# sunkafei/coffeedb

Hardware: AMD Instinct MI355X
Metric: sa_build_GiB_per_s (higher is better)
Workload: dtype u64

## Files before the change

### coffeedb_amd/csrc/debug_segsort.hip

```cpp
#include <cstdio>
#include <cstring>
#include <mutex>
#include <string>
#include <vector>

#include "../../include/coffeedb_gpu.h"
#include "index_impl.h"
#include "radix_sort.h"

using namespace cdb;

namespace {

std::mutex g_err_mu;
std::string g_err;

template <typename F>
int guarded_hook(const char* who, F&& f) {
    const int rc = guarded_call(g_err_mu, g_err, std::forward<F>(f));
    if (rc != CDB_OK) {
        std::lock_guard<std::mutex> g(g_err_mu);
        std::fprintf(stderr, "%s: %s\n", who, g_err.c_str());
    }
    return rc;
// ... 73 lines not shown
        CallStream cs(device);
        hipStream_t s = cs.s;
        StreamScope sscope(s);
        if (!rs_atomic_rank_ok(s)) throw InternalError("cdb_debug_segsort: needs the one-atomic ranking (internal)");
        const uint32_t cell_tiles_max = tiles + (form == CDB_DEBUG_SEGSORT_TOP_FIRST ? nb * 256u : 0u);
        Guarded k[2], v[2], w[2], eout, ehi, flags;
        for (int q = 0; q < 2; ++q) {
            k[q].alloc(n, 4, s);
            v[q].alloc(n, 4, s);
            w[q].alloc(n, 2, s);
        }
        eout.alloc(n, packed ? 4 : 8, s);
        ehi.alloc(n, 1, s);
        flags.alloc(n, 1, s);
        CDB_HIP(hipMemcpyAsync(k[0].ptr<uint32_t>(), k32, n * 4, hipMemcpyHostToDevice, s));
        CDB_HIP(hipMemcpyAsync(v[0].ptr<uint32_t>(), v32, n * 4, hipMemcpyHostToDevice, s));
        CDB_HIP(hipMemcpyAsync(w[0].ptr<uint16_t>(), w16, n * 2, hipMemcpyHostToDevice, s));
        DevBuf d_segs, d_tile_seg, d_hist, d_starts, edges;
        d_segs.alloc((size_t)nb * sizeof(SegInfo));
        CDB_HIP(hipMemcpyAsync(d_segs.p, segs.data(), (size_t)nb * sizeof(SegInfo), hipMemcpyHostToDevice, s));
        d_tile_seg.alloc((size_t)tiles * sizeof(uint32_t));
        d_hist.alloc((size_t)nb * 8 * 256 * sizeof(uint64_t));
        d_starts.alloc((size_t)nb * 8 * 256 * sizeof(uint64_t));
        edges.alloc((size_t)cell_tiles_max * 256 * sizeof(SegEdge));
        hipLaunchKernelGGL(rs_seg_tilemap_kernel, dim3((unsigned)ceil_div(tiles, 256u)), dim3(256), 0, s, (const SegInfo*)d_segs.as<SegInfo>(), nb, tiles,
                           d_tile_seg.as<uint32_t>());
        SegFinalArgs fin;
        if (packed) {
            fin.elo = eout.ptr<uint32_t>();
            fin.ehi = ehi.ptr<uint8_t>();
        } else {
            fin.eout = eout.ptr<uint64_t>();
        }
        fin.flags = flags.ptr<uint8_t>();
        fin.edges = edges.as<SegEdge>();
        fin.hi_shift = 8;
        fin.low_bits = 8;
        fin.kbase = 2;
        fin.kmagic = 0;
        if (carry) {
            fin.hi_mask = (1u << ehb) - 1u;
            fin.carry_mask = (1u << carry) - 1u;
            fin.carry_shift = 8 + ehb;
        }
        RadixWorkspace ws;
        ws.allow_group = true;
        Profiler prof;
        TopFirstWork tfw;
        uint32_t ncell = 0;
        if (form == CDB_DEBUG_SEGSORT_TOP_FIRST) {
            tfw.alloc(nb * 256u, cell_tiles_max);
            rs_top_first_fin(fin, ehb);
            ncell = radix_sort_top_first<uint16_t>(s, ws, prof, k[0].ptr<uint32_t>(), k[1].ptr<uint32_t>(), v[0].ptr<uint32_t>(), v[1].ptr<uint32_t>(),
                                                   w[0].ptr<uint16_t>(), w[1].ptr<uint16_t>(), n, (const SegInfo*)d_segs.as<SegInfo>(), segs.data(),
                                                   (const uint32_t*)d_tile_seg.as<uint32_t>(), nb, tiles, d_hist.as<unsigned long long>(),
                                                   d_starts.as<unsigned long long>(), tfw, fin, nullptr);
        } else {
            CDB_HIP(hipMemsetAsync(d_hist.p, 0, (size_t)nb * 8 * 256 * sizeof(uint64_t), s));
            hipLaunchKernelGGL((rs_seg_hist_kernel<uint16_t>), dim3((unsigned)ceil_div(tiles, (uint32_t)RS_MSD_HIST_TILES)), dim3(1024), 0, s,
                               (const uint32_t*)k[0].ptr<uint32_t>(), (const uint16_t*)w[0].ptr<uint16_t>(), 1, 5, (const uint32_t*)d_tile_seg.as<uint32_t>(),
                               (const SegInfo*)d_segs.as<SegInfo>(), tiles, d_hist.as<unsigned long long>());
            radix_sort_segmented<uint16_t>(s, ws, prof, k[0].ptr<uint32_t>(), k[1].ptr<uint32_t>(), v[0].ptr<uint32_t>(), v[1].ptr<uint32_t>(),
                                           w[0].ptr<uint16_t>(), w[1].ptr<uint16_t>(), n, (const SegInfo*)d_segs.as<SegInfo>(),
                                           (const uint32_t*)d_tile_seg.as<uint32_t>(), nb, tiles, (const unsigned long long*)d_hist.as<unsigned long long>(),
                                           d_starts.as<unsigned long long>(), 32, 1, fin, nullptr);
        }
        CDB_HIP(hipStreamSynchronize(s));
        radix_check_error(s, ws);
        if (packed) {
            std::vector<uint32_t> lo(n);
            std::vector<uint8_t> hi(n);
            CDB_HIP(hipMemcpyAsync(lo.data(), eout.ptr<uint32_t>(), n * 4, hipMemcpyDeviceToHost, s));
            CDB_HIP(hipMemcpyAsync(hi.data(), ehi.ptr<uint8_t>(), n, hipMemcpyDeviceToHost, s));
            CDB_HIP(hipStreamSynchronize(s));
            for (uint64_t i = 0; i < n; ++i) out_entries[i] = ((uint64_t)hi[i] << 32) | lo[i];
        } else {
            CDB_HIP(hipMemcpyAsync(out_entries, eout.ptr<uint64_t>(), n * 8, hipMemcpyDeviceToHost, s));
        }
        CDB_HIP(hipMemcpyAsync(out_flags, flags.ptr<uint8_t>(), n, hipMemcpyDeviceToHost, s));
// ... 17 lines not shown
```

### coffeedb_amd/csrc/radix_pass.h

```cpp
#pragma once
#include <cstdlib>

#include "common.h"

namespace cdb {

constexpr uint64_t RS_VAL_MASK = (1ull << 54) - 1;
constexpr uint32_t RS_SPIN_LIMIT_GROUPED = 1u << 18;
constexpr uint32_t RS_SPIN_LIMIT_PLAIN = 1u << 22;
constexpr int RS_GROUP = 8;

struct NoVal {};

__device__ __forceinline__ uint64_t rs_ld_status(const uint64_t* p) {
    return __hip_atomic_load(p, __ATOMIC_RELAXED, __HIP_MEMORY_SCOPE_AGENT);
}
__device__ __forceinline__ void rs_st_status(uint64_t* p, uint64_t v) {
    __hip_atomic_store(p, v, __ATOMIC_RELAXED, __HIP_MEMORY_SCOPE_AGENT);
}

template <int IPT_, bool REUSE_, bool EARLYV_, int NT_ = 256, bool NONTEMP_ = false, int MINW_ = 1, int ABL_ = 0,
          int LB_ = 1, bool DMA_ = false, bool ATOMRANK_ = false, bool TICKET_ = true, int LOAD_ = 0, int GROUP_ = 0>
struct RsCfg {
    static constexpr int GROUP = GROUP_;
    static constexpr int LOAD = LOAD_;
    static constexpr bool TICKET = TICKET_;
// ... 93 lines not shown
struct SegShrinkArgs : SegArgs {
    uint8_t* wout8 = nullptr;
};
struct SegEdge {
    unsigned long long first, last;
    unsigned long long pos;
    uint32_t cnt, pad;
};
struct SegFinalArgs : SegArgs {
    uint64_t* eout = nullptr;
    uint32_t* elo = nullptr;
    uint8_t* ehi = nullptr;
    uint8_t* flags = nullptr;
    SegEdge* edges = nullptr;
    int hi_shift = 0;
    int low_bits = 0;
    uint32_t kbase = 2;
    unsigned long long kmagic = 0;
    uint32_t hi_mask = 0xFFFFFFFFu;
    uint32_t carry_mask = 0;
    int carry_shift = 0;
};

struct SegFinalKeepArgs : SegArgs {
    uint8_t* flags = nullptr;
    SegEdge* edges = nullptr;
    int low_bits = 0;
    uint32_t kbase = 2;
    unsigned long long kmagic = 0;
    unsigned long long* tile_sums = nullptr;
    uint32_t sums_tile = 1;
    unsigned long long msd_m = 0;
};

struct SegFinalKeepMsdArgs : SegFinalKeepArgs {};

__device__ __forceinline__ uint64_t rs_pack_key(const uint32_t* __restrict__ s_words, uint32_t li, int nsym, uint32_t base,
                                                uint32_t rem) {
    const uint32_t wi = li >> 2, sel = li & 3u;
    const uint32_t b2 = base * base, b3 = b2 * base;
    const uint32_t pw[5] = {1u, base, b2, b3, b3 * base};
    uint64_t kk = 0;
    uint32_t lo = s_words[wi];
#pragma unroll
    for (int w = 0; w < 4; ++w) {
        const int q = 4 * w;
// ... 14 lines not shown

__device__ __forceinline__ uint64_t rs_doc_upper(const uint64_t* __restrict__ doc_start, uint64_t lo, uint64_t hi,
                                                 uint64_t p) {
    while (lo < hi) {
        const uint64_t mid = lo + (hi - lo + 1) / 2;
        if (doc_start[mid] <= p) lo = mid; else hi = mid - 1;
    }
    return lo;
}

template <typename K_, typename V_, typename Cfg_, typename Gen_, typename W_, typename Seg_>
struct RsTraits {
    using K = K_;
    using V = V_;
    using Cfg = Cfg_;
    using Gen = Gen_;
    using W = W_;
    using Seg = Seg_;
    static constexpr bool GEN = !std::is_same<Gen, NoGen>::value;
    static constexpr bool SEG = !std::is_same<Seg, NoSeg>::value;
    static constexpr bool FINAL = std::is_same<Seg, SegFinalArgs>::value;
    static constexpr bool KEEPM = std::is_same<Seg, SegFinalKeepMsdArgs>::value;
    static constexpr bool KEEP = std::is_same<Seg, SegFinalKeepArgs>::value || KEEPM;
    static constexpr bool FLAGS = FINAL || KEEP;
    static constexpr bool SHRINK = std::is_same<Seg, SegShrinkArgs>::value;
    static constexpr bool HAS_V = !std::is_same<V, NoVal>::value;
    static constexpr bool HAS_W = !std::is_same<W, NoVal>::value;
    using WS = typename std::conditional<HAS_W, W, uint8_t>::type;
    using VS = typename std::conditional<HAS_V, V, uint32_t>::type;
    static constexpr int IPT = Cfg::IPT;
    static constexpr bool REUSE = Cfg::REUSE && HAS_V;
    static constexpr bool EARLYV = (Cfg::EARLYV || REUSE) && HAS_V;
    static constexpr int NT = Cfg::NT;
    static constexpr int NW = NT / 64;
    static constexpr bool NTM = Cfg::NONTEMP;
    static constexpr int TILE = NT * IPT;
    static constexpr int WCHUNK = 64 * IPT;
    static constexpr size_t STAGE_K = sizeof(K) * TILE;
    static constexpr size_t STAGE_V = HAS_V ? sizeof(VS) * TILE : 0;
    static constexpr size_t STAGE_BYTES = REUSE ? (STAGE_K > STAGE_V ? STAGE_K : STAGE_V) : STAGE_K + STAGE_V;
    static constexpr bool GM_PAIR = std::is_same<Gen, TextGenPair>::value;
    static constexpr bool GM_REC = std::is_same<Gen, TextGenRec>::value;
    static constexpr bool BLK = GEN && sizeof(K) == 4 && sizeof(VS) == 4 && IPT == 16 && (NT == 1024 || NT == 512);
    static constexpr uint32_t GEN_TEXTB = ((TILE + RS_GEN_LOOK + 15) / 16) * 16;
    static constexpr uint32_t GEN_DOCS = 1024;
    static constexpr uint32_t GEN_SLOTS = 320;
    static constexpr size_t GEN_BYTES = BLK ? GEN_TEXTB + 512 + GEN_DOCS * 8 + GEN_SLOTS : 16;
    static constexpr uint32_t MAP_OFF = GEN_TEXTB;
    static constexpr uint32_t DOC_OFF = GEN_TEXTB + 512;
    static constexpr uint32_t DOC_CAP = BLK ? GEN_DOCS : (uint32_t)((STAGE_BYTES - DOC_OFF) / 8);
    static constexpr uint32_t SLOT_OFF = GEN_TEXTB + 512 + GEN_DOCS * 8;
    static constexpr bool W32G = GEN && HAS_W && sizeof(WS) == 4;
    static constexpr bool AUX_LDS = HAS_W && !W32G && !KEEPM;
    static constexpr size_t AUX_ELEMS = AUX_LDS ? TILE : 1;
    static constexpr bool LOAD_W = HAS_W && !KEEPM;
    static constexpr bool DMA_PATH = !GEN && Cfg::DMA && HAS_V && EARLYV && sizeof(K) == 8 && (IPT % 4) == 0;

    static_assert(!SHRINK || (std::is_same<W, uint16_t>::value && Cfg::REUSE && !std::is_same<V, NoVal>::value), "shrinking pass: u16 aux words, shared staging");
    static_assert(!SEG || (!GEN && !Cfg::DMA), "segmented passes: materialised records");
    static_assert(!FLAGS || Cfg::REUSE || KEEPM, "flag-writing passes: shared staging (the MSD-first last pass also runs with keys and values staged at once)");
    static_assert(!HAS_W || KEEPM || (Cfg::REUSE && HAS_V && !Cfg::DMA), "the auxiliary byte needs the shared-staging configuration");
    static_assert(!(GM_PAIR || GM_REC) || (BLK && HAS_W), "pair / records generators: 16 Ki tiles with an auxiliary word");
    static_assert(!GEN || EARLYV, "generator pass needs early values");
    static_assert(!GEN || STAGE_BYTES >= (size_t)TILE + RS_GEN_LOOK + 2048, "staging buffer too small for the text tile");
};
template <typename T>
__device__ __forceinline__ uint32_t rs_group_flag(const typename T::Seg& seg, bool head, bool tail, uint64_t kc, uint64_t slot,
                                                  uint32_t carry) {
    uint32_t f = head ? 1u : 0u;
    if (!(head && tail)) {
        const bool exhausted = seg.kmagic ? (kc - __umul64hi(kc, seg.kmagic) * seg.kbase) == 0
                                          : (kc & (uint64_t)(seg.kbase - 1u)) == 0;
        if (!exhausted) f |= 2u;
    }
    f |= carry;
    if (!(T::FINAL && (RS_SEG_ABL & 1))) seg.flags[slot] = (uint8_t)f;
    if constexpr (T::KEEP) {
        if ((f & 2u) && seg.tile_sums) {
            atomicAdd(seg.tile_sums + 2 * (slot / seg.sums_tile), 1ull);
            if (f & 1u) atomicAdd(seg.tile_sums + 2 * (slot / seg.sums_tile) + 1, 1ull);
        }
    }
// ... 63 lines not shown
        sg = seg.tile_seg ? seg.tile_seg[tile] : 0u;
        si = seg.segs[sg];
        tile0 = si.tile_begin;
        base = si.begin + (tile - tile0) * T::TILE;
        seg_n = si.end;
        if constexpr (T::KEEPM) ktop = (uint64_t)si.top * seg.msd_m;
    } else if constexpr (Cfg::GROUP > 0) {
        if (base >= n) return;
    }
    const uint32_t valid = (uint32_t)((seg_n - base) < (uint64_t)T::TILE ? (seg_n - base) : (uint64_t)T::TILE);
    if (s_bad) {
        if constexpr (T::GEN) {
            if (gen.tile_base) return;
        }
        if (tid < 256) rs_st_status(status + tile * 256 + tid, ((uint64_t)epoch << 56) | (2ull << 54));
        return;
    }

    K key[T::IPT];
    VS val[T::EARLYV ? T::IPT : 1];
    WS aux[T::HAS_W ? T::IPT : 1] = {};
    uint32_t gdig[T::GM_REC ? T::IPT / 4 : 1] = {};
    auto digit_of = [&](K k, WS a) -> uint32_t {
        if constexpr (T::HAS_W) {
            if (aux_shift >= 0) return ((uint32_t)a >> aux_shift) & dmask;
        }
        return (uint32_t)(k >> shift) & dmask;
    };
    const uint32_t wbase = wave * T::WCHUNK + lane;
    if constexpr (T::GEN) {
        unsigned char* const gbuf = T::BLK ? s_gen : s_stage;
        uint8_t* s_text = gbuf;
        uint16_t* s_map = reinterpret_cast<uint16_t*>(gbuf + T::MAP_OFF);
        uint64_t* s_docs = reinterpret_cast<uint64_t*>(gbuf + T::DOC_OFF);
        constexpr bool PRELOAD = T::BLK;
        uint4 tw0 = make_uint4(0, 0, 0, 0), tw1 = make_uint4(0, 0, 0, 0);
        bool tw0_ok = false, tw1_ok = false;
        if constexpr (PRELOAD) {
            const uint64_t g0 = base + (uint64_t)tid * 16, g1 = base + (uint64_t)T::TILE + (uint64_t)tid * 16;
            tw0_ok = gen.padded ? (g0 < n + RS_GEN_LOOK) : (g0 + 16 <= n);
            tw1_ok = (uint32_t)tid * 16 < (uint32_t)RS_GEN_LOOK && (gen.padded ? (g1 < n + RS_GEN_LOOK) : (g1 + 16 <= n));
            if (tw0_ok) tw0 = *reinterpret_cast<const uint4*>(gen.text + g0);
            if (tw1_ok) tw1 = *reinterpret_cast<const uint4*>(gen.text + g1);
        }
        const uint64_t dlo = gen.tile_doc[tile], dhi = gen.tile_doc[tile + 1];
        for (int i = tid; i < 256; i += T::NT) s_map[i] = gen.symmap[i];
        if constexpr (T::GM_REC) {
// ... 398 lines not shown
                atomicAdd(err + 1, (uint32_t)used);
                atomicAdd(err + 2, 1u);
            }
            p -= used;
            if (used == 0) {
                __builtin_amdgcn_s_sleep(1);
                if (++spins > (Cfg::GROUP > 0 ? RS_SPIN_LIMIT_GROUPED : RS_SPIN_LIMIT_PLAIN)) {
                    atomicExch(err, 1u);
                    break;
                }
            } else {
                spins = 0;
            }
        }
        rs_st_status(my, tag | (2ull << 54) | (excl + real));
    }
    uint64_t dstart = 0;
    if (tid < 256) {
        if constexpr (T::SEG) dstart = (uint64_t)digit_start[(size_t)sg * seg.start_stride + d];
        else dstart = (uint64_t)digit_start[d];
        s_gbase[d] = (Cfg::ABL & 2) ? base : (prebased ? pre : dstart + excl) - (uint64_t)tstart;
    }
    __syncthreads();
    if constexpr (T::FLAGS) {
        if (tid < 256) {
            SegEdge e;
            e.first = e.last = 0;
            e.pos = dstart + excl;
            e.cnt = (uint32_t)real;
            e.pad = 0;
            if (real) {
                const uint64_t lmask = (1ull << seg.low_bits) - 1ull;
                const uint32_t a = tstart, b = tstart + (uint32_t)real - 1u;
                if constexpr (T::KEEPM) {
                    e.first = ktop + (uint64_t)s_keys[a];
                    e.last = ktop + (uint64_t)s_keys[b];
                } else {
                    e.first = ((uint64_t)s_keys[a] << seg.low_bits) | ((uint64_t)s_aux[T::HAS_W ? a : 0] & lmask);
                    e.last = ((uint64_t)s_keys[b] << seg.low_bits) | ((uint64_t)s_aux[T::HAS_W ? b : 0] & lmask);
                }
            }
            seg.edges[tile * 256 + d] = e;
        }
    }

    if constexpr (!T::REUSE) {
#pragma unroll
        for (int j = 0; j < T::IPT; ++j) {
            const uint32_t i = j * T::NT + tid;
            if (i < valid) {
                const K k = s_keys[i];
                const uint32_t dd = (uint32_t)(k >> shift) & dmask;
                const uint64_t dst = s_gbase[dd] + i;
                if constexpr (T::KEEPM) {
                    bool head = true, tail = true;
                    if (i > 0) head = s_keys[i - 1] != k;
                    if (i + 1 < valid) tail = s_keys[i + 1] != k;
                    const uint64_t kf = ktop + (uint64_t)k;
                    rs_group_flag<T>(seg, head, tail, kf, dst, 0u);
                    rs_store<T::NTM>(kout + dst, (K)(kf >> 8));
                    if constexpr (T::HAS_W) rs_store<T::NTM>(wout + dst, (W)(kf & 0xFFu));
                    rs_store<T::NTM>(vout + dst, (V)s_vals[i]);
                    continue;
                }
                if (!T::GEN || kout) rs_store<T::NTM>(kout + dst, k);
                if constexpr (T::HAS_V) rs_store<T::NTM>(vout + dst, (V)s_vals[i]);
            }
        }
    } else {
        uint8_t dig[T::IPT];
#pragma unroll
        for (int j = 0; j < T::IPT; ++j) {
            const uint32_t i = j * T::NT + tid;
            dig[j] = 0;
            if (i < valid) {
                const K k = s_keys[i];
                uint32_t dd;
                if constexpr (T::KEEPM) dd = (uint32_t)(k >> shift) & dmask;
                else dd = digit_of(k, s_aux[T::HAS_W ? i : 0]);
                if constexpr (T::GM_REC) dd = (uint32_t)s_gen[i];
                dig[j] = (uint8_t)dd;
                if constexpr (T::FLAGS) {
                    const uint32_t lmask = seg.low_bits >= 32 ? 0xFFFFFFFFu : (1u << seg.low_bits) - 1u;
                    uint32_t ac = 0;
                    if constexpr (!T::KEEPM) ac = (uint32_t)s_aux[T::HAS_W ? i : 0] & lmask;
                    bool head = true, tail = true;
                    bool cmp = true;
                    if constexpr (T::FINAL) cmp = !(RS_SEG_ABL & 4);
                    if constexpr (T::KEEPM) {
// ... 78 lines not shown
```

### coffeedb_amd/csrc/radix_sort.h

```cpp
#pragma once
#include <cstdlib>

#include "common.h"
#include "radix_pass.h"

namespace cdb {

constexpr int RS_MAX_PASSES = 16;

template <typename K>
__global__ __launch_bounds__(256) void rs_hist_kernel(const K* __restrict__ keys, uint64_t n, int begin_bit,
                                                      int npass, int dbits, uint32_t last_mask,
                                                      unsigned long long* __restrict__ ghist) {
    __shared__ uint32_t sh[RS_MAX_PASSES * 256];
    for (int i = threadIdx.x; i < npass * 256; i += 256) sh[i] = 0;
    __syncthreads();
    const uint64_t stride = (uint64_t)gridDim.x * 256;
    for (uint64_t i = (uint64_t)blockIdx.x * 256 + threadIdx.x; i < n; i += stride) {
        const K k = keys[i];
#pragma unroll
        for (int p = 0; p < RS_MAX_PASSES; ++p) {
            if (p < npass) {
                uint32_t d = (uint32_t)(k >> (begin_bit + dbits * p)) & ((1u << dbits) - 1u);
                if (p == npass - 1) d &= last_mask;
// ... 51 lines not shown
        if (r >= (1u << 24) || (b2 - 1) * r >= (1ull << 32)) break;
        bool ok = true;
        for (uint64_t a = 0; a < b2 && ok; ++a) ok = ((a * r) >> sh) == a / span;
        if (ok) {
            gen.pair_span = span;
            gen.pair_r = (uint32_t)r;
            gen.pair_s = sh;
            return true;
        }
    }
    return false;
}

static __global__ __launch_bounds__(256) void rs_tiledoc_kernel(const uint64_t* __restrict__ doc_start, uint64_t ndocs,
                                                                uint64_t n, uint64_t tile_elems, uint64_t tiles,
                                                                uint64_t* __restrict__ tile_doc) {
    const uint64_t t = (uint64_t)blockIdx.x * 256 + threadIdx.x;
    if (t > tiles) return;
    const uint64_t p = t * tile_elems < n ? t * tile_elems : n - 1;
    tile_doc[t] = rs_doc_upper(doc_start, 0, ndocs - 1, p);
}


static __global__ __launch_bounds__(256) void rs_seg_edge_fix_kernel(const SegEdge* __restrict__ edges, const uint32_t* __restrict__ tile_seg,
                                                                     const SegInfo* __restrict__ segs, uint32_t tiles,
                                                                     uint8_t* __restrict__ flags, uint32_t kbase, unsigned long long kmagic,
                                                                     unsigned long long* __restrict__ tile_sums = nullptr,
                                                                     uint32_t sums_tile = 1, const uint32_t* __restrict__ err = nullptr) {
    const uint32_t t = blockIdx.x, d = threadIdx.x;
    if (t >= tiles) return;
    if (err && *err) return;
    const SegEdge e = edges[(size_t)t * 256 + d];
    if (!e.cnt) return;
    const SegInfo si = segs[tile_seg ? tile_seg[t] : 0u];
    const uint32_t t0 = si.tile_begin;
    if (t == t0) return;
    uint32_t lo = t0, hi = t;
    if (edges[(size_t)(t - 1) * 256 + d].pos < e.pos) {
        lo = t - 1;
    } else {
        if (edges[(size_t)t0 * 256 + d].pos >= e.pos) return;
        hi = t - 1;
        while (hi - lo > 1) {
            const uint32_t mid = lo + (hi - lo) / 2;
            if (edges[(size_t)mid * 256 + d].pos < e.pos) lo = mid; else hi = mid;
        }
    }
    const SegEdge pe = edges[(size_t)lo * 256 + d];
    if (pe.last != e.first) return;
    const bool exhausted = kmagic ? (e.first - __umul64hi(e.first, kmagic) * kbase) == 0 : (e.first & (uint64_t)(kbase - 1u)) == 0;
    auto change = [&](unsigned long long slot, uint32_t clear, uint32_t set) {
        const uintptr_t a = reinterpret_cast<uintptr_t>(flags + slot);
        unsigned int* w = reinterpret_cast<unsigned int*>(a & ~(uintptr_t)3);
        const uint32_t sh = 8u * (uint32_t)(a & 3u);
        uint32_t before, after;
        if (clear) {
            before = (atomicAnd(w, ~(clear << sh)) >> sh) & 0xFFu;
            after = before & ~clear;
        } else {
            before = (atomicOr(w, set << sh) >> sh) & 0xFFu;
            after = before | set;
        }
        if (tile_sums && before != after) {
            const long long da = (long long)((after >> 1) & 1u) - (long long)((before >> 1) & 1u);
            const long long db = (long long)((after >> 1) & after & 1u) - (long long)((before >> 1) & before & 1u);
            unsigned long long* ts = tile_sums + 2 * (slot / sums_tile);
            if (da) atomicAdd(ts, (unsigned long long)da);
            if (db) atomicAdd(ts + 1, (unsigned long long)db);
        }
    };
    const unsigned long long sb = rs_seg_rotated(si, e.pos), sa_ = rs_seg_rotated(si, e.pos - 1);
    change(sb, 1u, 0u);
    if (!exhausted) {
        change(sb, 0u, 2u);
        change(sa_, 0u, 2u);
    }
}

static __global__ __launch_bounds__(256) void rs_lane_order_probe_kernel(uint32_t* __restrict__ bad) {
    __shared__ uint32_t cnt[4][256];
    __shared__ uint32_t ref[4][256];
    const int tid = threadIdx.x, lane = tid & 63, wave = tid >> 6;
    for (int i = tid; i < 4 * 256; i += 256) {
        (&cnt[0][0])[i] = 0;
        (&ref[0][0])[i] = 0;
    }
    __syncthreads();
    const uint64_t lt_mask = (1ull << lane) - 1ull;
    uint32_t wrong = 0;
    for (uint32_t r = 0; r < 64; ++r) {
        uint32_t h = (blockIdx.x * 64u + r) * 256u + (uint32_t)tid;
        h ^= h >> 16; h *= 0x7feb352du; h ^= h >> 15; h *= 0x846ca68bu; h ^= h >> 16;
        const uint32_t mode = blockIdx.x & 3u;
        const uint32_t d = mode == 0 ? 7u : mode == 1 ? (h & 1u) * 64u : mode == 2 ? (h & 15u) * 4u : (h & 255u);
        const uint32_t got = atomicAdd(&cnt[wave][d], 1u);
        uint64_t m = ~0ull;
#pragma unroll
        for (int b = 0; b < 8; ++b) {
            const bool bit = (d >> b) & 1u;
// ... 409 lines not shown

static __global__ __launch_bounds__(256) void rs_seg_digit_start_kernel(const unsigned long long* __restrict__ hist,
                                                                        const SegInfo* __restrict__ segs, int npass,
                                                                        unsigned long long* __restrict__ starts) {
    __shared__ unsigned long long s[256];
    const uint32_t g = blockIdx.x;
    const int t = threadIdx.x;
    const unsigned long long b0 = segs[g].begin;
    for (int p = 0; p < npass; ++p) {
        const unsigned long long c = hist[((size_t)g * 8 + p) * 256 + t];
        s[t] = c;
        __syncthreads();
        for (int off = 1; off < 256; off <<= 1) {
            const unsigned long long v = t >= off ? s[t - off] : 0;
            __syncthreads();
            s[t] += v;
            __syncthreads();
        }
        starts[((size_t)g * 8 + p) * 256 + t] = b0 + s[t] - c;
        __syncthreads();
    }
}

template <typename W>
void radix_sort_segmented(hipStream_t s, RadixWorkspace& ws, Profiler& prof, uint32_t* k0, uint32_t* k1, uint32_t* v0, uint32_t* v1,
                          W* w0, W* w1, uint64_t m, const SegInfo* d_segs, const uint32_t* d_tile_seg, uint32_t nseg, uint32_t tiles,
                          const unsigned long long* d_hist, unsigned long long* d_starts, int key_bits, int lead, SegFinalArgs fin,
                          SortStats* stats) {
    if (!rs_atomic_rank_ok(s)) throw InternalError("radix_sort_segmented: needs the one-atomic ranking (internal)");
    const int kpass = (int)ceil_div((uint64_t)key_bits, 8);
    const int npass = kpass + lead;
    if (npass < 1 || npass > 8 || kpass < 1) throw InternalError("radix_sort_segmented: unsupported pass count (internal)");
    const int last_bits = key_bits - 8 * (kpass - 1);
    const uint32_t last_mask = (1u << last_bits) - 1u;
    ws.prepare((uint64_t)tiles * RS_SEG_TILE, RS_SEG_TILE, s);
    hipLaunchKernelGGL(rs_seg_digit_start_kernel, dim3(nseg), dim3(256), 0, s, d_hist, d_segs, npass, d_starts);
    SegArgs sa;
    sa.tile_seg = d_tile_seg;
    sa.segs = d_segs;
    sa.tiles = tiles;
    sa.start_stride = 8 * 256;
    static_cast<SegArgs&>(fin) = sa;
    uint32_t* kb[2] = {k0, k1};
    uint32_t* vb[2] = {v0, v1};
    W* wb[2] = {w0, w1};
    int cur = 0;
    const char* wn = sizeof(W) == 1 ? "_w8" : (sizeof(W) == 2 ? "_w16" : "_w32");
    const size_t rec = 8 + sizeof(W);
    for (int p = 0; p < npass; ++p) {
        const uint32_t dmask = p == npass - 1 ? last_mask : 0xFFu;
        const int shift = 8 * (p - lead);
        const int aux_shift = p < lead ? 8 * p : -1;
        const unsigned long long* dstart = d_starts + (size_t)p * 256;
        int t = prof.begin(s);
        if (p == npass - 1) {
            rs_launch_pass_ordered<RsBig<>, W>(s, ws, tiles, kb[cur], kb[cur ^ 1], vb[cur], vb[cur ^ 1], m, shift, dmask, dstart, NoGen(), wb[cur],
                                               wb[cur ^ 1], aux_shift, fin);
            prof.end(t, (std::string("rs_seg_final") + wn + "_t16384").c_str(), m * (rec + (fin.elo ? 6 : 9)), s);
        } else {
            rs_launch_pass_ordered<RsBig<>, W>(s, ws, tiles, kb[cur], kb[cur ^ 1], vb[cur], vb[cur ^ 1], m, shift, dmask, dstart, NoGen(), wb[cur],
                                               wb[cur ^ 1], aux_shift, sa);
            prof.end(t, (std::string("rs_seg_k32_v32") + wn + "_t16384").c_str(), 2 * m * rec, s);
        }
        cur ^= 1;
        if (stats) stats->passes_run++;
    }
    int t = prof.begin(s);
    hipLaunchKernelGGL(rs_seg_edge_fix_kernel, dim3(tiles), dim3(256), 0, s, (const SegEdge*)fin.edges, d_tile_seg, d_segs, tiles,
                       fin.flags, fin.kbase, fin.kmagic, (unsigned long long*)nullptr, 1u, (const uint32_t*)ws.err_ptr());
    prof.end(t, "rs_seg_edge_fix", (uint64_t)tiles * 256 * sizeof(SegEdge), s);
    CDB_HIP(hipGetLastError());
}

constexpr int RS_MSD_HIST_TILES = 32;

template <typename W, bool KEYS = true>
__global__ __launch_bounds__(1024) void rs_seg_hist_kernel(const uint32_t* __restrict__ keys, const W* __restrict__ aux, int lead, int npass,
                                                           const uint32_t* __restrict__ tile_seg, const SegInfo* __restrict__ segs,
                                                           uint32_t tiles, unsigned long long* __restrict__ hist) {
    constexpr int NC = 4, HC = 8 * 256 + 64 / NC;
    __shared__ uint32_t sh4[NC * HC];
    const int tid = threadIdx.x;
    uint32_t* const sh = sh4 + (tid & (NC - 1)) * HC;
    const uint32_t t0 = blockIdx.x * RS_MSD_HIST_TILES;
    const uint32_t t1 = t0 + RS_MSD_HIST_TILES < tiles ? t0 + RS_MSD_HIST_TILES : tiles;
    uint32_t cur = ~0u;
    auto flush = [&]() {
        __syncthreads();
        if (cur != ~0u)
            for (int i = tid; i < npass * 256; i += 1024) {
                uint32_t c = 0;
#pragma unroll
                for (int q = 0; q < NC; ++q) c += sh4[q * HC + i];
// ... 98 lines not shown
            if (tiles > 0xFFFFFFFFull) throw InternalError("radix_sort_top_first: tile count (internal)");
        }
        if (at != h_segs[b].end) throw InternalError("radix_sort_top_first: top-digit counts do not add up to the bucket (internal)");
    }
    return (uint32_t)tiles;
}
inline void rs_check_cells(const std::vector<SegInfo>& cells, uint32_t tiles, const SegInfo* h_segs, uint32_t nseg) {
    uint64_t t = 0;
    size_t c = 0;
    for (uint32_t b = 0; b < nseg; ++b) {
        unsigned long long at = h_segs[b].begin;
        while (c < cells.size() && cells[c].begin == at && at < h_segs[b].end) {
            const SegInfo& ci = cells[c];
            if (ci.end <= ci.begin || ci.end > h_segs[b].end || (uint64_t)ci.tile_begin != t || ci.rot_b)
                throw InternalError("radix_sort_top_first: cell table (internal)");
            t += (ci.end - ci.begin + (uint64_t)RS_SEG_TILE - 1) / (uint64_t)RS_SEG_TILE;
            at = ci.end;
            ++c;
        }
        if (at != h_segs[b].end) throw InternalError("radix_sort_top_first: cells do not cover their bucket (internal)");
    }
    if (c != cells.size() || t != (uint64_t)tiles) throw InternalError("radix_sort_top_first: cell tiles (internal)");
}
inline void rs_top_first_fin(SegFinalArgs& fin, int ehb) {
    fin.hi_shift = 0;
    fin.low_bits = 0;
    fin.hi_mask = (1u << ehb) - 1u;
    fin.carry_shift = ehb;
}
template <typename W>
uint32_t radix_sort_top_first(hipStream_t s, RadixWorkspace& ws, Profiler& prof, uint32_t* k0, uint32_t* k1, uint32_t* v0, uint32_t* v1,
                                     W* w0, W* w1, uint64_t m, const SegInfo* d_segs, const SegInfo* h_segs, const uint32_t* d_tile_seg,
                                     uint32_t nseg, uint32_t tiles, unsigned long long* d_hist, unsigned long long* d_starts, TopFirstWork& tw,
                                     SegFinalArgs fin, SortStats* stats) {
    static_assert(std::is_same<W, uint16_t>::value, "top digit first: (u32, u32, u16) records");
    if (!rs_atomic_rank_ok(s)) throw InternalError("radix_sort_top_first: needs the one-atomic ranking (internal)");
    for (uint32_t b = 0; b < nseg; ++b)
        if (h_segs[b].rot_b) throw InternalError("radix_sort_top_first: rotated bucket (internal)");
    CDB_HIP(hipMemsetAsync(d_hist, 0, (size_t)nseg * 8 * 256 * sizeof(uint64_t), s));
    int t = prof.begin(s);
    hipLaunchKernelGGL((rs_seg_hist_kernel<W, false>), dim3((unsigned)ceil_div(tiles, (uint32_t)RS_MSD_HIST_TILES)), dim3(1024), 0, s,
                       (const uint32_t*)k0, (const W*)w0, 1, 1, d_tile_seg, d_segs, tiles, d_hist);
    prof.end(t, "rs_seg_hist_top", m * sizeof(W), s);
    tw.h_hist.resize((size_t)nseg * 8 * 256);
    CDB_HIP(hipMemcpyAsync(tw.h_hist.data(), d_hist, tw.h_hist.size() * sizeof(uint64_t), hipMemcpyDeviceToHost, s));
    CDB_HIP(hipStreamSynchronize(s));
    hipLaunchKernelGGL(rs_seg_digit_start_kernel, dim3(nseg), dim3(256), 0, s, (const unsigned long long*)d_hist, d_segs, 1, d_starts);
    ws.prepare((uint64_t)tiles * RS_SEG_TILE, RS_SEG_TILE, s);
    SegShrinkArgs sh;
    sh.tile_seg = d_tile_seg;
    sh.segs = d_segs;
    sh.tiles = tiles;
    sh.start_stride = 8 * 256;
    sh.wout8 = reinterpret_cast<uint8_t*>(w1);
    t = prof.begin(s);
    rs_launch_pass_ordered<RsBig<>, W>(s, ws, tiles, k0, k1, v0, v1, m, -8, 0xFFu, (const unsigned long long*)d_starts, NoGen(), w0, w1, 0, sh);
    prof.end(t, "rs_seg_top_w16_t16384", m * (10 + 9), s);
    if (stats) stats->passes_run++;
    const uint32_t ctiles = rs_top_first_cells(h_segs, nseg, tw.h_hist.data(), tw.h_cells);
    rs_check_cells(tw.h_cells, ctiles, h_segs, nseg);
    CDB_HIP(hipStreamSynchronize(s));
    const uint32_t ncell = (uint32_t)tw.h_cells.size();
    if (ncell == 0 || ncell > tw.cell_cap || ctiles > tw.tile_cap) throw InternalError("radix_sort_top_first: cell scratch (internal)");
    CDB_HIP(hipMemcpyAsync(tw.cells.p, tw.h_cells.data(), (size_t)ncell * sizeof(SegInfo), hipMemcpyHostToDevice, s));
    hipLaunchKernelGGL(rs_seg_tilemap_kernel, dim3((unsigned)ceil_div(ctiles, 256u)), dim3(256), 0, s, (const SegInfo*)tw.cells.as<SegInfo>(), ncell,
                       ctiles, tw.tile_seg.as<uint32_t>());
    uint8_t* const b0 = reinterpret_cast<uint8_t*>(w0);
    uint8_t* const b1 = reinterpret_cast<uint8_t*>(w1);
    CDB_HIP(hipMemsetAsync(tw.hist.p, 0, (size_t)ncell * 8 * 256 * sizeof(uint64_t), s));
    t = prof.begin(s);
    hipLaunchKernelGGL((rs_seg_hist_kernel<uint8_t>), dim3((unsigned)ceil_div(ctiles, (uint32_t)RS_MSD_HIST_TILES)), dim3(1024), 0, s, (const uint32_t*)k1,
                       (const uint8_t*)b1, 0, 4, (const uint32_t*)tw.tile_seg.as<uint32_t>(), (const SegInfo*)tw.cells.as<SegInfo>(), ctiles,
                       tw.hist.as<unsigned long long>());
    prof.end(t, "rs_seg_hist_cells", m * sizeof(uint32_t), s);
    radix_sort_segmented<uint8_t>(s, ws, prof, k1, k0, v1, v0, b1, b0, m, (const SegInfo*)tw.cells.as<SegInfo>(), (const uint32_t*)tw.tile_seg.as<uint32_t>(), ncell,
                                  ctiles, (const unsigned long long*)tw.hist.as<unsigned long long>(), tw.starts.as<unsigned long long>(), 32, 0, fin, stats);
    return ncell;
}

constexpr int RS_GEN8_TILE = 8192;
constexpr uint32_t RS_TB_ROWS = 256;
static __global__ __launch_bounds__(256) void rs_tilecol_sum_kernel(const uint32_t* __restrict__ counts, uint32_t rows, const uint16_t* __restrict__ src_col,
                                                                    unsigned long long* __restrict__ partial) {
    const uint32_t d = threadIdx.x, b = blockIdx.x;
    const uint32_t c = src_col ? (uint32_t)src_col[d] : d;
    const uint32_t r0 = b * RS_TB_ROWS, r1 = r0 + RS_TB_ROWS < rows ? r0 + RS_TB_ROWS : rows;
    unsigned long long sum = 0;
    if (c < 256u)
        for (uint32_t r = r0; r < r1; ++r) sum += counts[(size_t)r * 256 + c];
    partial[(size_t)b * 256 + d] = sum;
}
static __global__ __launch_bounds__(1024) void rs_tilecol_total_kernel(const unsigned long long* __restrict__ partial, uint32_t blocks,
                                                                       unsigned long long* __restrict__ totals) {
    __shared__ unsigned long long s_q[4][256];
    const uint32_t d = threadIdx.x & 255u, g = threadIdx.x >> 8;
    const uint32_t per = (blocks + 3u) / 4u;
    const uint32_t b0 = g * per, b1 = b0 + per < blocks ? b0 + per : blocks;
    unsigned long long sum = 0;
// ... 251 lines not shown
```

### coffeedb_amd/csrc/sa_build.hip

```cpp
#include <algorithm>
#include <chrono>
#include <cmath>
#include <cstdlib>
#include <cstring>

#include "sa_build_phases.h"
#include "records_sweep.h"
#include "vl_code.h"

#ifndef RS_GATHER_ABL
#define RS_GATHER_ABL 0
#endif

namespace cdb {

double now_ms() {
    using namespace std::chrono;
    return duration<double, std::milli>(steady_clock::now().time_since_epoch()).count();
}

namespace {

constexpr int KG_TILE = 2048;
constexpr int KG_LOOK = 64;
// ... 1597 lines not shown
        uint32_t *kbp[2], *ebp[2];
        const int dead = bpass & 1;
        for (int q = 0; q < 2; ++q) {
            if (fuse_rec) {
                kb[q] = std::move(rf.fr_kv[q]);
                kbp[q] = kb[q].as<uint32_t>();
                if (out.packed_out) {
                    eb[q] = std::move(rf.fr_e[q]);
                    ebp[q] = eb[q].as<uint32_t>();
                } else {
                    ebp[q] = kbp[q] + max_elems;
                }
                wb[q] = std::move(rf.fr_w[q]);
                if (wb[q].bytes < max_elems * (top_first && q == 1 ? 1 : sizeof(W))) throw InternalError("run_segmented: aux buffer of the fused form (internal)");
                continue;
            } else {
                kb[q].alloc(max_elems * sizeof(uint32_t));
                eb[q].alloc(max_elems * sizeof(uint32_t));
                kbp[q] = kb[q].as<uint32_t>();
                ebp[q] = eb[q].as<uint32_t>();
            }
            wb[q].alloc(max_elems * (top_first && q == 1 ? 1 : sizeof(W)));
        }
        edges.alloc((size_t)cell_tiles_max * 256 * sizeof(SegEdge));
        if (top_first) tfw.alloc(max_gb * 256u, cell_tiles_max);
        d_starts.alloc((size_t)max_gb * 8 * 256 * sizeof(uint64_t));
        d_bh2.alloc((size_t)max_gb * 8 * 256 * sizeof(uint64_t));
        d_segs.alloc((size_t)nb * sizeof(SegInfo));
        tile_seg.alloc((size_t)max_tiles * sizeof(uint32_t));
        cell_off.alloc((size_t)max_cells * sizeof(uint32_t));
        lists.alloc(groups.size() * 16 * sizeof(uint32_t));
        d_items2.alloc((size_t)max_items * sizeof(BucketItem));
        st.alloc_ms += now_ms() - ta;
        CDB_HIP(hipMemcpyAsync(d_segs.p, h_segs.data(), (size_t)nb * sizeof(SegInfo), hipMemcpyHostToDevice, s));
        CDB_HIP(hipMemsetAsync(lists.p, 0, groups.size() * 16 * sizeof(uint32_t), s));
        const unsigned long long* bnd = br.d_bounds.as<unsigned long long>();
        for (size_t gi = 0; gi < groups.size(); ++gi) {
            const Group& g = groups[gi];
            const uint32_t gb = g.b1 - g.b0;
            uint32_t* list_len = lists.as<uint32_t>() + gi * 16;
            uint32_t* tickets = list_len + 8;
            if (fuse_rec && !sweep_fused) {
                {
                    hipLaunchKernelGGL(rs_seg_tilemap_kernel, dim3((unsigned)ceil_div(g.tiles, 256)), dim3(256), 0, s,
                                       (const SegInfo*)(d_segs.as<SegInfo>() + g.b0), gb, g.tiles, tile_seg.as<uint32_t>());
                    TextGen rg{text, doc_start, al.d_symmap.as<uint16_t>(), D, (int)ix.bits, bbase, nsym, 0, ix.text_padded};
                    rg.slotmap = d_slotmap.as<uint8_t>();
// ... 67 lines not shown
            SegFinalArgs fin;
            if (pack_seg) {
                fin.elo = E.as<uint32_t>() + g.gstart;
                fin.ehi = out.sa_hi_buf.as<uint8_t>() + g.gstart;
            } else if (out.packed_out) {
                fin.elo = kbp[dead] + g.gstart;
                fin.ehi = out.sa_hi_buf.as<uint8_t>() + g.gstart;
            } else {
                fin.eout = (fuse_rec ? kb[dead].as<uint64_t>() : E.as<uint64_t>()) + g.gstart;
            }
            fin.flags = out.flags.as<uint8_t>() + g.gstart;
            fin.edges = edges.as<SegEdge>();
            fin.hi_shift = blow;
            fin.low_bits = blow;
            fin.kbase = br.fbase;
            fin.kmagic = br.bmagic;
            if (carry) {
                fin.hi_mask = (1u << ehb) - 1u;
                fin.carry_mask = (1u << carry) - 1u;
                fin.carry_shift = blow + ehb;
            }
            if constexpr (std::is_same<W, uint16_t>::value) {
                if (top_first) {
                    rs_top_first_fin(fin, ehb);
                    st.top_first_cells += radix_sort_top_first(s, ix.rws, ix.prof, kbp[0], kbp[1], ebp[0], ebp[1], wb[0].as<W>(), wb[1].as<W>(),
                                                               g.elems, (const SegInfo*)(d_segs.as<SegInfo>() + g.b0), h_segs.data() + g.b0,
                                                               (const uint32_t*)tile_seg.as<uint32_t>(), gb, g.tiles, d_bh2.as<unsigned long long>(),
                                                               d_starts.as<unsigned long long>(), tfw, fin, &ss);
                    st.bucket_groups++;
                    continue;
                }
            }
            radix_sort_segmented<W>(s, ix.rws, ix.prof, kbp[0], kbp[1], ebp[0], ebp[1], wb[0].as<W>(), wb[1].as<W>(), g.elems,
                                    (const SegInfo*)(d_segs.as<SegInfo>() + g.b0), (const uint32_t*)tile_seg.as<uint32_t>(), gb,
                                    g.tiles, (const unsigned long long*)d_bh2.as<unsigned long long>(),
                                    d_starts.as<unsigned long long>(), rf.bbits - blow, lowb, fin, &ss);
            st.bucket_groups++;
        }
        CDB_HIP(hipStreamSynchronize(s));
        if (sweep_rec || sweep_fused) ix.tbw.base.release();
        if (fuse_rec) E = std::move(kb[dead]);
        if (pack_seg) out.packed_out = true;
        st.segmented = 1;
    }
}

template <typename V, typename I>
void run_per_bucket(Index& ix, const Alphabet& al, const KeyPlan& kp, const Buckets& bk, const RecordForm& rf, const BucketRecords& br,
                    DevBuf& E, InitialSort& out, SortStats& ss) {
    hipStream_t s = ix.stream;
    const uint64_t n = ix.size;
// ... 524 lines not shown
```

Baseline: 32.77.

## Specialise top-first last cell pass with compact 16-byte edge records

Adds a dedicated final-pass variant for the top-digit-first segmented sort over cells, with its own argument struct and a 16-byte edge record that packs position and count and stores 32-bit first/last keys. The cell final pass writes flags and entries through a simplified path with fixed base-2 keys: no rotation, no magic-division exhaustion check, and the digit comes directly from the key. The edge-fix kernel is templated to read the compact records. The aim is less edge-record memory traffic and simpler per-element work in the last pass, at the cost of new limits (positions below 2^48, tiles up to 16384, at most 8 entry bits) that are checked on the host.

Result: faster. 33.51, median of 6 (+2.3%).

```diff
diff --git a/coffeedb_amd/csrc/debug_segsort.hip b/coffeedb_amd/csrc/debug_segsort.hip
--- a/coffeedb_amd/csrc/debug_segsort.hip
+++ b/coffeedb_amd/csrc/debug_segsort.hip
@@ -119,7 +119,7 @@
         d_tile_seg.alloc((size_t)tiles * sizeof(uint32_t));
         d_hist.alloc((size_t)nb * 8 * 256 * sizeof(uint64_t));
         d_starts.alloc((size_t)nb * 8 * 256 * sizeof(uint64_t));
-        edges.alloc((size_t)cell_tiles_max * 256 * sizeof(SegEdge));
+        edges.alloc((size_t)cell_tiles_max * 256 * (form == CDB_DEBUG_SEGSORT_TOP_FIRST ? sizeof(SegCellEdge) : sizeof(SegEdge)));
         hipLaunchKernelGGL(rs_seg_tilemap_kernel, dim3((unsigned)ceil_div(tiles, 256u)), dim3(256), 0, s, (const SegInfo*)d_segs.as<SegInfo>(), nb, tiles,
                            d_tile_seg.as<uint32_t>());
         SegFinalArgs fin;
@@ -147,11 +147,11 @@
         uint32_t ncell = 0;
         if (form == CDB_DEBUG_SEGSORT_TOP_FIRST) {
             tfw.alloc(nb * 256u, cell_tiles_max);
-            rs_top_first_fin(fin, ehb);
+            const SegFinalCellArgs cfin = rs_top_first_fin(fin, ehb);
             ncell = radix_sort_top_first<uint16_t>(s, ws, prof, k[0].ptr<uint32_t>(), k[1].ptr<uint32_t>(), v[0].ptr<uint32_t>(), v[1].ptr<uint32_t>(),
                                                    w[0].ptr<uint16_t>(), w[1].ptr<uint16_t>(), n, (const SegInfo*)d_segs.as<SegInfo>(), segs.data(),
                                                    (const uint32_t*)d_tile_seg.as<uint32_t>(), nb, tiles, d_hist.as<unsigned long long>(),
-                                                   d_starts.as<unsigned long long>(), tfw, fin, nullptr);
+                                                   d_starts.as<unsigned long long>(), tfw, cfin, nullptr);
         } else {
             CDB_HIP(hipMemsetAsync(d_hist.p, 0, (size_t)nb * 8 * 256 * sizeof(uint64_t), s));
             hipLaunchKernelGGL((rs_seg_hist_kernel<uint16_t>), dim3((unsigned)ceil_div(tiles, (uint32_t)RS_MSD_HIST_TILES)), dim3(1024), 0, s,
diff --git a/coffeedb_amd/csrc/radix_pass.h b/coffeedb_amd/csrc/radix_pass.h
--- a/coffeedb_amd/csrc/radix_pass.h
+++ b/coffeedb_amd/csrc/radix_pass.h
@@ -2,6 +2,7 @@
 #include <cstdlib>
 
 #include "common.h"
+#include "seg_cell_edge.h"
 
 namespace cdb {
 
@@ -141,6 +142,17 @@
     int carry_shift = 0;
 };
 
+struct SegFinalCellArgs : SegArgs {
+    uint64_t* eout = nullptr;
+    uint32_t* elo = nullptr;
+    uint8_t* ehi = nullptr;
+    uint8_t* flags = nullptr;
+    SegCellEdge* edges = nullptr;
+    uint32_t hi_mask = 0xFFu;
+    uint32_t carry_mask = 0;
+    int carry_shift = 0;
+};
+
 struct SegFinalKeepArgs : SegArgs {
     uint8_t* flags = nullptr;
     SegEdge* edges = nullptr;
@@ -201,7 +213,8 @@
     static constexpr bool FINAL = std::is_same<Seg, SegFinalArgs>::value;
     static constexpr bool KEEPM = std::is_same<Seg, SegFinalKeepMsdArgs>::value;
     static constexpr bool KEEP = std::is_same<Seg, SegFinalKeepArgs>::value || KEEPM;
-    static constexpr bool FLAGS = FINAL || KEEP;
+    static constexpr bool CELL = std::is_same<Seg, SegFinalCellArgs>::value;
+    static constexpr bool FLAGS = FINAL || KEEP || CELL;
     static constexpr bool SHRINK = std::is_same<Seg, SegShrinkArgs>::value;
     static constexpr bool HAS_V = !std::is_same<V, NoVal>::value;
     static constexpr bool HAS_W = !std::is_same<W, NoVal>::value;
@@ -237,6 +250,8 @@
 
     static_assert(!SHRINK || (std::is_same<W, uint16_t>::value && Cfg::REUSE && !std::is_same<V, NoVal>::value), "shrinking pass: u16 aux words, shared staging");
     static_assert(!SEG || (!GEN && !Cfg::DMA), "segmented passes: materialised records");
+    static_assert(!CELL || (std::is_same<K, uint32_t>::value && std::is_same<V, uint32_t>::value && std::is_same<W, uint8_t>::value && (IPT % 4) == 0),
+                  "last pass over cells: (u32, u32, u8) records");
     static_assert(!FLAGS || Cfg::REUSE || KEEPM, "flag-writing passes: shared staging (the MSD-first last pass also runs with keys and values staged at once)");
     static_assert(!HAS_W || KEEPM || (Cfg::REUSE && HAS_V && !Cfg::DMA), "the auxiliary byte needs the shared-staging configuration");
     static_assert(!(GM_PAIR || GM_REC) || (BLK && HAS_W), "pair / records generators: 16 Ki tiles with an auxiliary word");
@@ -346,7 +361,7 @@
     WS aux[T::HAS_W ? T::IPT : 1] = {};
     uint32_t gdig[T::GM_REC ? T::IPT / 4 : 1] = {};
     auto digit_of = [&](K k, WS a) -> uint32_t {
-        if constexpr (T::HAS_W) {
+        if constexpr (T::HAS_W && !T::CELL) {
             if (aux_shift >= 0) return ((uint32_t)a >> aux_shift) & dmask;
         }
         return (uint32_t)(k >> shift) & dmask;
@@ -791,7 +806,12 @@
         s_gbase[d] = (Cfg::ABL & 2) ? base : (prebased ? pre : dstart + excl) - (uint64_t)tstart;
     }
     __syncthreads();
-    if constexpr (T::FLAGS) {
+    if constexpr (T::CELL) {
+        if (tid < 256) {
+            const uint32_t a = tstart, b = tstart + (uint32_t)real - 1u;
+            seg.edges[tile * 256 + d] = seg_cell_edge_pack(real ? s_keys[a] : 0u, real ? s_keys[b] : 0u, dstart + excl, (uint32_t)real);
+        }
+    } else if constexpr (T::FLAGS) {
         if (tid < 256) {
             SegEdge e;
             e.first = e.last = 0;
@@ -834,6 +854,46 @@
                 }
                 if (!T::GEN || kout) rs_store<T::NTM>(kout + dst, k);
                 if constexpr (T::HAS_V) rs_store<T::NTM>(vout + dst, (V)s_vals[i]);
+            }
+        }
+    } else if constexpr (T::CELL) {
+        uint32_t dig4[T::IPT / 4] = {}, aux4[T::IPT / 4] = {};
+#pragma unroll
+        for (int j = 0; j < T::IPT; ++j) {
+            const uint32_t i = j * T::NT + tid;
+            if (i < valid) {
+                const uint32_t k = s_keys[i];
+                const uint32_t dd = (k >> shift) & dmask;
+                const uint32_t a = (uint32_t)s_aux[i];
+                dig4[j >> 2] |= dd << (8 * (j & 3));
+                aux4[j >> 2] |= a << (8 * (j & 3));
+                bool head = true, tail = true;
+                if (!(RS_SEG_ABL & 4)) {
+                    if (i > 0) head = s_keys[i - 1] != k;
+                    if (i + 1 < valid) tail = s_keys[i + 1] != k;
+                }
+                uint32_t f = head ? 1u : 0u;
+                if (!(head && tail) && (k & 1u)) f |= 2u;
+                f |= ((a >> seg.carry_shift) & seg.carry_mask) << 2;
+                if (!(RS_SEG_ABL & 1)) seg.flags[s_gbase[dd] + i] = (uint8_t)f;
+            }
+        }
+        __syncthreads();
+#pragma unroll
+        for (int j = 0; j < T::IPT; ++j) s_vals[rank[j]] = val[j];
+        __syncthreads();
+#pragma unroll
+        for (int j = 0; j < T::IPT; ++j) {
+            const uint32_t i = j * T::NT + tid;
+            if (i < valid && !(RS_SEG_ABL & 2)) {
+                const unsigned long long slot = s_gbase[(dig4[j >> 2] >> (8 * (j & 3))) & 0xFFu] + i;
+                const uint32_t hi32 = (aux4[j >> 2] >> (8 * (j & 3))) & seg.hi_mask;
+                if (seg.elo) {
+                    seg.elo[slot] = (uint32_t)s_vals[i];
+                    seg.ehi[slot] = (uint8_t)hi32;
+                } else {
+                    seg.eout[slot] = ((uint64_t)hi32 << 32) | (uint64_t)s_vals[i];
+                }
             }
         }
     } else {
diff --git a/coffeedb_amd/csrc/radix_sort.h b/coffeedb_amd/csrc/radix_sort.h
--- a/coffeedb_amd/csrc/radix_sort.h
+++ b/coffeedb_amd/csrc/radix_sort.h
@@ -97,33 +97,42 @@
 }
 
 
-static __global__ __launch_bounds__(256) void rs_seg_edge_fix_kernel(const SegEdge* __restrict__ edges, const uint32_t* __restrict__ tile_seg,
-                                                                     const SegInfo* __restrict__ segs, uint32_t tiles,
-                                                                     uint8_t* __restrict__ flags, uint32_t kbase, unsigned long long kmagic,
-                                                                     unsigned long long* __restrict__ tile_sums = nullptr,
-                                                                     uint32_t sums_tile = 1, const uint32_t* __restrict__ err = nullptr) {
+__device__ __forceinline__ unsigned long long rs_edge_pos(const SegEdge& e) { return e.pos; }
+__device__ __forceinline__ uint32_t rs_edge_cnt(const SegEdge& e) { return e.cnt; }
+__device__ __forceinline__ unsigned long long rs_edge_first(const SegEdge& e) { return e.first; }
+__device__ __forceinline__ unsigned long long rs_edge_last(const SegEdge& e) { return e.last; }
+__device__ __forceinline__ unsigned long long rs_edge_pos(const SegCellEdge& e) { return seg_cell_edge_pos(e.pos_cnt); }
+__device__ __forceinline__ uint32_t rs_edge_cnt(const SegCellEdge& e) { return seg_cell_edge_cnt(e.pos_cnt); }
+__device__ __forceinline__ unsigned long long rs_edge_first(const SegCellEdge& e) { return e.first; }
+__device__ __forceinline__ unsigned long long rs_edge_last(const SegCellEdge& e) { return e.last; }
+template <typename E>
+__device__ __forceinline__ void rs_seg_edge_fix_body(const E* __restrict__ edges, const uint32_t* __restrict__ tile_seg,
+                                                     const SegInfo* __restrict__ segs, uint32_t tiles, uint8_t* __restrict__ flags, uint32_t kbase,
+                                                     unsigned long long kmagic, unsigned long long* __restrict__ tile_sums, uint32_t sums_tile,
+                                                     const uint32_t* __restrict__ err) {
+    constexpr bool CELL = std::is_same<E, SegCellEdge>::value;
     const uint32_t t = blockIdx.x, d = threadIdx.x;
     if (t >= tiles) return;
     if (err && *err) return;
-    const SegEdge e = edges[(size_t)t * 256 + d];
-    if (!e.cnt) return;
+    const E e = edges[(size_t)t * 256 + d];
+    if (!rs_edge_cnt(e)) return;
+    const unsigned long long epos = rs_edge_pos(e), efirst = rs_edge_first(e);
     const SegInfo si = segs[tile_seg ? tile_seg[t] : 0u];
     const uint32_t t0 = si.tile_begin;
     if (t == t0) return;
     uint32_t lo = t0, hi = t;
-    if (edges[(size_t)(t - 1) * 256 + d].pos < e.pos) {
+    if (rs_edge_pos(edges[(size_t)(t - 1) * 256 + d]) < epos) {
         lo = t - 1;
     } else {
-        if (edges[(size_t)t0 * 256 + d].pos >= e.pos) return;
+        if (rs_edge_pos(edges[(size_t)t0 * 256 + d]) >= epos) return;
         hi = t - 1;
         while (hi - lo > 1) {
             const uint32_t mid = lo + (hi - lo) / 2;
-            if (edges[(size_t)mid * 256 + d].pos < e.pos) lo = mid; else hi = mid;
-        }
-    }
-    const SegEdge pe = edges[(size_t)lo * 256 + d];
-    if (pe.last != e.first) return;
-    const bool exhausted = kmagic ? (e.first - __umul64hi(e.first, kmagic) * kbase) == 0 : (e.first & (uint64_t)(kbase - 1u)) == 0;
+            if (rs_edge_pos(edges[(size_t)mid * 256 + d]) < epos) lo = mid; else hi = mid;
+        }
+    }
+    if (rs_edge_last(edges[(size_t)lo * 256 + d]) != efirst) return;
+    const bool exhausted = kmagic ? (efirst - __umul64hi(efirst, kmagic) * kbase) == 0 : (efirst & (uint64_t)(kbase - 1u)) == 0;
     auto change = [&](unsigned long long slot, uint32_t clear, uint32_t set) {
         const uintptr_t a = reinterpret_cast<uintptr_t>(flags + slot);
         unsigned int* w = reinterpret_cast<unsigned int*>(a & ~(uintptr_t)3);
@@ -144,12 +153,24 @@
             if (db) atomicAdd(ts + 1, (unsigned long long)db);
         }
     };
-    const unsigned long long sb = rs_seg_rotated(si, e.pos), sa_ = rs_seg_rotated(si, e.pos - 1);
+    const unsigned long long sb = CELL ? epos : rs_seg_rotated(si, epos), sa_ = CELL ? epos - 1 : rs_seg_rotated(si, epos - 1);
     change(sb, 1u, 0u);
     if (!exhausted) {
         change(sb, 0u, 2u);
         change(sa_, 0u, 2u);
     }
+}
+static __global__ __launch_bounds__(256) void rs_seg_edge_fix_kernel(const SegEdge* __restrict__ edges, const uint32_t* __restrict__ tile_seg,
+                                                                     const SegInfo* __restrict__ segs, uint32_t tiles,
+                                                                     uint8_t* __restrict__ flags, uint32_t kbase, unsigned long long kmagic,
+                                                                     unsigned long long* __restrict__ tile_sums = nullptr,
+                                                                     uint32_t sums_tile = 1, const uint32_t* __restrict__ err = nullptr) {
+    rs_seg_edge_fix_body(edges, tile_seg, segs, tiles, flags, kbase, kmagic, tile_sums, sums_tile, err);
+}
+static __global__ __launch_bounds__(256) void rs_seg_edge_fix_cell_kernel(const SegCellEdge* __restrict__ edges, const uint32_t* __restrict__ tile_seg,
+                                                                          const SegInfo* __restrict__ segs, uint32_t tiles,
+                                                                          uint8_t* __restrict__ flags, const uint32_t* __restrict__ err) {
+    rs_seg_edge_fix_body(edges, tile_seg, segs, tiles, flags, 2u, 0ull, (unsigned long long*)nullptr, 1u, err);
 }
 
 static __global__ __launch_bounds__(256) void rs_lane_order_probe_kernel(uint32_t* __restrict__ bad) {
@@ -605,15 +626,21 @@
     }
 }
 
-template <typename W>
+template <typename W, typename Fin = SegFinalArgs>
 void radix_sort_segmented(hipStream_t s, RadixWorkspace& ws, Profiler& prof, uint32_t* k0, uint32_t* k1, uint32_t* v0, uint32_t* v1,
                           W* w0, W* w1, uint64_t m, const SegInfo* d_segs, const uint32_t* d_tile_seg, uint32_t nseg, uint32_t tiles,
-                          const unsigned long long* d_hist, unsigned long long* d_starts, int key_bits, int lead, SegFinalArgs fin,
+                          const unsigned long long* d_hist, unsigned long long* d_starts, int key_bits, int lead, Fin fin,
                           SortStats* stats) {
+    constexpr bool CELL = std::is_same<Fin, SegFinalCellArgs>::value;
     if (!rs_atomic_rank_ok(s)) throw InternalError("radix_sort_segmented: needs the one-atomic ranking (internal)");
     const int kpass = (int)ceil_div((uint64_t)key_bits, 8);
     const int npass = kpass + lead;
     if (npass < 1 || npass > 8 || kpass < 1) throw InternalError("radix_sort_segmented: unsupported pass count (internal)");
+    if constexpr (CELL) {
+        static_assert(std::is_same<W, uint8_t>::value, "last pass over cells: byte-wide aux words");
+        if (lead != 0 || key_bits != 32 || fin.hi_mask > 0xFFu) throw InternalError("radix_sort_segmented: cell form (internal)");
+        seg_cell_edge_check_limits(m, RS_SEG_TILE);
+    }
     const int last_bits = key_bits - 8 * (kpass - 1);
     const uint32_t last_mask = (1u << last_bits) - 1u;
     ws.prepare((uint64_t)tiles * RS_SEG_TILE, RS_SEG_TILE, s);
@@ -649,9 +676,15 @@
         if (stats) stats->passes_run++;
     }
     int t = prof.begin(s);
-    hipLaunchKernelGGL(rs_seg_edge_fix_kernel, dim3(tiles), dim3(256), 0, s, (const SegEdge*)fin.edges, d_tile_seg, d_segs, tiles,
-                       fin.flags, fin.kbase, fin.kmagic, (unsigned long long*)nullptr, 1u, (const uint32_t*)ws.err_ptr());
-    prof.end(t, "rs_seg_edge_fix", (uint64_t)tiles * 256 * sizeof(SegEdge), s);
+    if constexpr (CELL) {
+        hipLaunchKernelGGL(rs_seg_edge_fix_cell_kernel, dim3(tiles), dim3(256), 0, s, (const SegCellEdge*)fin.edges, d_tile_seg, d_segs, tiles,
+                           fin.flags, (const uint32_t*)ws.err_ptr());
+        prof.end(t, "rs_seg_edge_fix", (uint64_t)tiles * 256 * sizeof(SegCellEdge), s);
+    } else {
+        hipLaunchKernelGGL(rs_seg_edge_fix_kernel, dim3(tiles), dim3(256), 0, s, (const SegEdge*)fin.edges, d_tile_seg, d_segs, tiles,
+                           fin.flags, fin.kbase, fin.kmagic, (unsigned long long*)nullptr, 1u, (const uint32_t*)ws.err_ptr());
+        prof.end(t, "rs_seg_edge_fix", (uint64_t)tiles * 256 * sizeof(SegEdge), s);
+    }
     CDB_HIP(hipGetLastError());
 }
 
@@ -796,17 +829,24 @@
     }
     if (c != cells.size() || t != (uint64_t)tiles) throw InternalError("radix_sort_top_first: cell tiles (internal)");
 }
-inline void rs_top_first_fin(SegFinalArgs& fin, int ehb) {
-    fin.hi_shift = 0;
-    fin.low_bits = 0;
-    fin.hi_mask = (1u << ehb) - 1u;
-    fin.carry_shift = ehb;
+inline SegFinalCellArgs rs_top_first_fin(const SegFinalArgs& fin, int ehb) {
+    if (fin.kbase != 2 || fin.kmagic != 0 || ehb < 0 || ehb > 8) throw InternalError("radix_sort_top_first: variable-length keys, at most 8 entry bits in the aux byte (internal)");
+    SegFinalCellArgs c;
+    c.eout = fin.eout;
+    c.elo = fin.elo;
+    c.ehi = fin.ehi;
+    c.flags = fin.flags;
+    c.edges = reinterpret_cast<SegCellEdge*>(fin.edges);
+    c.hi_mask = (1u << ehb) - 1u;
+    c.carry_mask = fin.carry_mask;
+    c.carry_shift = ehb;
+    return c;
 }
 template <typename W>
 uint32_t radix_sort_top_first(hipStream_t s, RadixWorkspace& ws, Profiler& prof, uint32_t* k0, uint32_t* k1, uint32_t* v0, uint32_t* v1,
                                      W* w0, W* w1, uint64_t m, const SegInfo* d_segs, const SegInfo* h_segs, const uint32_t* d_tile_seg,
                                      uint32_t nseg, uint32_t tiles, unsigned long long* d_hist, unsigned long long* d_starts, TopFirstWork& tw,
-                                     SegFinalArgs fin, SortStats* stats) {
+                                     SegFinalCellArgs fin, SortStats* stats) {
     static_assert(std::is_same<W, uint16_t>::value, "top digit first: (u32, u32, u16) records");
     if (!rs_atomic_rank_ok(s)) throw InternalError("radix_sort_top_first: needs the one-atomic ranking (internal)");
     for (uint32_t b = 0; b < nseg; ++b)
@@ -847,7 +887,7 @@
                        (const uint8_t*)b1, 0, 4, (const uint32_t*)tw.tile_seg.as<uint32_t>(), (const SegInfo*)tw.cells.as<SegInfo>(), ctiles,
                        tw.hist.as<unsigned long long>());
     prof.end(t, "rs_seg_hist_cells", m * sizeof(uint32_t), s);
-    radix_sort_segmented<uint8_t>(s, ws, prof, k1, k0, v1, v0, b1, b0, m, (const SegInfo*)tw.cells.as<SegInfo>(), (const uint32_t*)tw.tile_seg.as<uint32_t>(), ncell,
+    radix_sort_segmented<uint8_t, SegFinalCellArgs>(s, ws, prof, k1, k0, v1, v0, b1, b0, m, (const SegInfo*)tw.cells.as<SegInfo>(), (const uint32_t*)tw.tile_seg.as<uint32_t>(), ncell,
                                   ctiles, (const unsigned long long*)tw.hist.as<unsigned long long>(), tw.starts.as<unsigned long long>(), 32, 0, fin, stats);
     return ncell;
 }
diff --git a/coffeedb_amd/csrc/sa_build.hip b/coffeedb_amd/csrc/sa_build.hip
--- a/coffeedb_amd/csrc/sa_build.hip
+++ b/coffeedb_amd/csrc/sa_build.hip
@@ -1643,7 +1643,7 @@
             }
             wb[q].alloc(max_elems * (top_first && q == 1 ? 1 : sizeof(W)));
         }
-        edges.alloc((size_t)cell_tiles_max * 256 * sizeof(SegEdge));
+        edges.alloc((size_t)cell_tiles_max * 256 * (top_first ? sizeof(SegCellEdge) : sizeof(SegEdge)));
         if (top_first) tfw.alloc(max_gb * 256u, cell_tiles_max);
         d_starts.alloc((size_t)max_gb * 8 * 256 * sizeof(uint64_t));
         d_bh2.alloc((size_t)max_gb * 8 * 256 * sizeof(uint64_t));
@@ -1757,11 +1757,11 @@
             }
             if constexpr (std::is_same<W, uint16_t>::value) {
                 if (top_first) {
-                    rs_top_first_fin(fin, ehb);
+                    const SegFinalCellArgs cfin = rs_top_first_fin(fin, ehb);
                     st.top_first_cells += radix_sort_top_first(s, ix.rws, ix.prof, kbp[0], kbp[1], ebp[0], ebp[1], wb[0].as<W>(), wb[1].as<W>(),
                                                                g.elems, (const SegInfo*)(d_segs.as<SegInfo>() + g.b0), h_segs.data() + g.b0,
                                                                (const uint32_t*)tile_seg.as<uint32_t>(), gb, g.tiles, d_bh2.as<unsigned long long>(),
-                                                               d_starts.as<unsigned long long>(), tfw, fin, &ss);
+                                                               d_starts.as<unsigned long long>(), tfw, cfin, &ss);
                     st.bucket_groups++;
                     continue;
                 }
diff --git a/coffeedb_amd/csrc/seg_cell_edge.h b/coffeedb_amd/csrc/seg_cell_edge.h
--- /dev/null
+++ b/coffeedb_amd/csrc/seg_cell_edge.h
@@ -0,0 +1,41 @@
+#pragma once
+#include <cstdint>
+#include <string>
+
+#include "errors.h"
+
+#if defined(__HIPCC__)
+#define CDB_CELL_EDGE_HD __host__ __device__ __forceinline__
+#else
+#define CDB_CELL_EDGE_HD inline
+#endif
+
+namespace cdb {
+
+constexpr int SEG_CELL_POS_BITS = 48;
+constexpr uint32_t SEG_CELL_CNT_MAX = 16384;
+constexpr unsigned long long SEG_CELL_POS_MASK = (1ull << SEG_CELL_POS_BITS) - 1ull;
+
+struct SegCellEdge {
+    uint32_t first, last;
+    unsigned long long pos_cnt;
+};
+static_assert(sizeof(SegCellEdge) == 16, "cell edge record: 16 bytes");
+
+CDB_CELL_EDGE_HD SegCellEdge seg_cell_edge_pack(uint32_t first, uint32_t last, unsigned long long pos, uint32_t cnt) {
+    SegCellEdge e;
+    e.first = first;
+    e.last = last;
+    e.pos_cnt = pos | ((unsigned long long)cnt << SEG_CELL_POS_BITS);
+    return e;
+}
+CDB_CELL_EDGE_HD unsigned long long seg_cell_edge_pos(unsigned long long pos_cnt) { return pos_cnt & SEG_CELL_POS_MASK; }
+CDB_CELL_EDGE_HD uint32_t seg_cell_edge_cnt(unsigned long long pos_cnt) { return (uint32_t)(pos_cnt >> SEG_CELL_POS_BITS); }
+
+inline void seg_cell_edge_check_limits(unsigned long long slots, unsigned long long tile) {
+    if (slots > (1ull << SEG_CELL_POS_BITS)) throw InternalError("cell edge record: output slot beyond 2^48 (internal)");
+    if (tile > (unsigned long long)SEG_CELL_CNT_MAX)
+        throw InternalError("cell edge record: a run of more than 16384 elements (internal)");
+}
+
+}
```
